# ZulutionAI/MoviiGen1.1

Measured on AMD Instinct MI355X. Metric: denoise-steps/sec, higher is better.
Workload: dtype bf16; 1 GPU; 14B T2V 1920x832x81f bf16 (the metric's configuration; BASELINE configs[2] shape); layers=40, parallelism=single, solver=unipc, weights=random N(0,0.02) bf16, seed 0

## Files before the change

### include/moviigen_hip.h

```cpp
#ifndef MOVIIGEN_HIP_H
#define MOVIIGEN_HIP_H

#include <stdint.h>

#ifdef __cplusplus
extern "C" {
#endif

#define MG_OK 0
#define MG_ERR_ARG (-1)
#define MG_ERR_SHAPE (-2)
#define MG_ERR_LAUNCH (-3)
#define MG_ERR_UNAVAILABLE (-4)
#define MG_ERR_COMM (-5)

const char* mg_version(void);
int mg_abi_version(void);


int mg_ln_modulate(const float* x, int64_t ldx, int64_t rows, int dim, const float* scale,
                   const float* shift, int add_one, float eps, int round_norm_bf16, void* out,
                   int out_f32, int64_t ldo, void* stream);

int64_t mg_step_resid_partials_bytes(void);
// ... 19 lines not shown

int mg_gemm_bf16(const uint16_t* A, int64_t lda, const uint16_t* W, int64_t ldw,
                 const float* bias, int64_t M, int N, int K, int epilogue, void* out,
                 int64_t ldo, const float* gate, void* stream);

int mg_quant_mxfp8_rows(const uint16_t* x, int64_t ldx, int64_t rows, int K, uint8_t* q, int64_t ldq,
                        uint8_t* scales, int64_t lds, void* stream);

int mg_gemm_mxfp8(const uint8_t* Aq, int64_t lda, const uint8_t* As, int64_t ldas, const uint8_t* Wq, int64_t ldw,
                  const uint8_t* Ws, int64_t ldws, const float* bias, int64_t M, int N, int K, int epilogue,
                  void* out, int64_t ldo, const float* gate, void* stream);

int mg_ln_modulate_mxfp8(const float* x, int64_t ldx, int64_t rows, int dim, const float* scale, const float* shift,
                         int add_one, float eps, int round_norm_bf16, uint16_t* out, int64_t ldo, uint8_t* q,
                         int64_t ldq, uint8_t* scales, int64_t lds, void* stream);

int mg_gemm_mxfp8_gelu_q(const uint8_t* Aq, int64_t lda, const uint8_t* As, int64_t ldas, const uint8_t* Wq, int64_t ldw,
                         const uint8_t* Ws, int64_t ldws, const float* bias, int64_t M, int N, int K, uint8_t* oq,
                         int64_t ldoq, uint8_t* oscales, int64_t ldos, void* stream);

int64_t mg_attn_workspace_bytes(void);
int mg_attn_fwd_bf16_hd128(const uint16_t* q, int64_t ldq, const uint16_t* kp, const uint16_t* vp,
                           uint16_t* o, int64_t ldo, int64_t Lq, int64_t Lk, int heads, float scale,
                           void* workspace, void* stream);

int mg_attn_fwd_bf16_hd128_lse(const uint16_t* q, int64_t ldq, const uint16_t* kp, const uint16_t* vp,
                               uint16_t* o, int64_t ldo, float* lse, int64_t Lq, int64_t Lk, int heads,
                               float scale, void* workspace, void* stream);

int mg_attn_fwd_bf16_hd128_prescaled(const uint16_t* q, int64_t ldq, const uint16_t* kp, const uint16_t* vp,
                                     uint16_t* o, int64_t ldo, float* lse, int64_t Lq, int64_t Lk, int heads,
                                     int reserve_cus, void* workspace, void* stream);

int mg_gate_residual_f32(float* x, int64_t ldx, const uint16_t* y, int64_t ldy, const float* gate, int64_t rows,
                         int dim, void* stream);


int mg_sp_pack_qkv_bf16(const uint16_t* q, int64_t ldq, const uint16_t* k, int64_t ldk, const uint16_t* v,
                        int64_t ldv, int64_t Lloc, int P, int cols_per_dest, int col0, int w, uint16_t* send,
                        void* stream);

int mg_sp_unpack_o_bf16(const uint16_t* recv, int64_t Lloc, int P, int cols_per_src, int col0, int w, uint16_t* o,
                        int64_t ldo, void* stream);

int mg_sp_copy_blocks_bf16(const uint16_t* src, int64_t s_blk, int64_t s_row, uint16_t* dst, int64_t d_blk,
                           int64_t d_row, int blocks, int64_t rows, int width, void* stream);


int mg_comm_unique_id(void* id128);
int mg_comm_create(const void* id128, int nranks, int rank, void** comm);
int mg_comm_destroy(void* comm);

int mg_sp_all_to_all(void* comm, const void* send, void* recv, int64_t bytes_per_peer, void* stream);

int mg_sp_all_to_all_4d_bf16(void* comm, const uint16_t* x, int64_t ldx, int64_t rows, int heads, int head_dim,
                             int seq_to_head, uint16_t* out, int64_t ldo, uint16_t* workspace, void* stream);

int mg_sp_all_gather(void* comm, const void* send, void* recv, int64_t bytes, void* stream);
int mg_shard_all_gather(void* comm, const void* shard, void* full, int64_t shard_bytes, void* stream);

int mg_attn_merge_f32(float* acc, int64_t lda, float* lse_acc, const uint16_t* part, int64_t ldp,
                      const float* lse_part, uint16_t* out, int64_t ldo, int64_t Lq, int heads, int first,
                      void* stream);

int mg_attn_fwd_bf16_generic(const uint16_t* q, int64_t ldq, const uint16_t* k, int64_t ldk,
                             const uint16_t* v, int64_t ldv, uint16_t* o, int64_t ldo, int64_t Lq,
// ... 112 lines not shown
```

### moviigen1.1_amd/csrc/attn_hd128.hip

```cpp
#include "common.h"
#include "../../include/moviigen_hip.h"

#define ATT_QB 256

__global__ __launch_bounds__(256) void pack_kv_kernel(const uint16_t* __restrict__ k, int64_t ldk,
                                                      const uint16_t* __restrict__ v, int64_t ldv, int64_t L,
                                                      uint16_t* __restrict__ kp, uint16_t* __restrict__ vp, int nt,
                                                      int korder) {
    __shared__ uint16_t tile[64][128 + 8];
    const int head = blockIdx.y, t = blockIdx.x;
    const int64_t k0 = (int64_t)t * 64;
    const int64_t tbase = ((int64_t)head * nt + t) * 8192;
    if (k) {
#pragma unroll
        for (int i = 0; i < 4; ++i) {
            const int id = threadIdx.x + i * 256;
            const int r = id >> 4, c = id & 15;
            u16x8_t u = {0, 0, 0, 0, 0, 0, 0, 0};
            if (k0 + r < L) u = *(const u16x8_t*)(k + (k0 + r) * ldk + head * 128 + c * 8);
            const int row = korder ? ((r & 32) | ((r & 4) << 2) | ((r & 24) >> 1) | (r & 3)) : r;
            *(u16x8_t*)(kp + tbase + c * 512 + row * 8) = u;
        }
    }
    if (v) {
#pragma unroll
        for (int i = 0; i < 4; ++i) {
            const int id = threadIdx.x + i * 256;
            const int r = id >> 4, c = id & 15;
            u16x8_t u = {0, 0, 0, 0, 0, 0, 0, 0};
            if (k0 + r < L) u = *(const u16x8_t*)(v + (k0 + r) * ldv + head * 128 + c * 8);
            *(u16x8_t*)&tile[r][c * 8] = u;
        }
        __syncthreads();
#pragma unroll
        for (int i = 0; i < 4; ++i) {
            const int id = threadIdx.x + i * 256;
            const int kc = id >> 7, d = id & 127;
            u16x8_t u;
#pragma unroll
            for (int j = 0; j < 8; ++j) u[j] = tile[kc * 8 + j][d];
            *(u16x8_t*)(vp + tbase + kc * 1024 + d * 8) = u;
        }
    }
}

#ifdef MG_AB_BUILD
int mg_attn_w64_launch(const uint16_t* q, int64_t ldq, const uint16_t* kp, const uint16_t* vp, uint16_t* o, int64_t ldo,
                       int64_t Lq, int64_t Lk, int heads, float c_log2, int nqb, float* lse, hipStream_t st);
#endif
int mg_attn_m16_launch(const uint16_t* q, int64_t ldq, const uint16_t* kp, const uint16_t* vp, uint16_t* o, int64_t ldo,
                       int64_t Lq, int64_t Lk, int heads, float c_log2, int prescaled, int nqb, float* lse, int reserve_cus,
                       unsigned* workspace, hipStream_t st);

#ifdef MG_AB_BUILD
static int g_attn_variant = 0;
extern "C" int mg_attn_set_variant(int v) {
    if (v != 0 && v != 3) return MG_ERR_ARG;
    g_attn_variant = v;
    return MG_OK;
}
#else
static constexpr int g_attn_variant = 0;
#endif

extern "C" int mg_pack_kv_bf16(const uint16_t* k, int64_t ldk, const uint16_t* v, int64_t ldv, int64_t L, int heads,
                               int head_dim, uint16_t* kp, uint16_t* vp, void* stream) {
    if ((!k && !v) || (k && !kp) || (v && !vp)) return MG_ERR_ARG;
    if (head_dim != 128 || heads <= 0 || L <= 0 || (k && (ldk & 7)) || (v && (ldv & 7))) return MG_ERR_SHAPE;
    const int nt = (int)((L + 63) / 64);
    hipLaunchKernelGGL(pack_kv_kernel, dim3(nt, heads), dim3(256), 0, (hipStream_t)stream, k, ldk, v, ldv, L, kp, vp,
                       nt, g_attn_variant == 3 ? 0 : 1);
    return mg_check_launch();
}

static int attn_fwd_impl(const uint16_t* q, int64_t ldq, const uint16_t* kp, const uint16_t* vp, uint16_t* o, int64_t ldo,
                         float* lse, int64_t Lq, int64_t Lk, int heads, float scale, int prescaled, int reserve_cus, void* workspace,
                         void* stream) {
    if (!q || !kp || !vp || !o) return MG_ERR_ARG;
    if ((uintptr_t)workspace & 7) return MG_ERR_SHAPE;
    if (Lq < 0 || Lk <= 0 || heads <= 0 || reserve_cus < 0) return MG_ERR_SHAPE;
    if ((ldq & 7) || (ldo & 3)) return MG_ERR_SHAPE;
    if (((uintptr_t)q & 15) || ((uintptr_t)kp & 15) || ((uintptr_t)vp & 15) || ((uintptr_t)o & 7)) return MG_ERR_SHAPE;
    if (Lq == 0) return MG_OK;
    const int64_t nqb64 = (Lq + ATT_QB - 1) / ATT_QB;
    if (nqb64 * heads > 0x7fffffffLL) return MG_ERR_SHAPE;
    const int nqb = (int)nqb64;
    const float c_log2 = scale * 1.4426950408889634f;
    hipStream_t st = (hipStream_t)stream;
#ifdef MG_AB_BUILD
    if (g_attn_variant == 3)
        return mg_attn_w64_launch(q, ldq, kp, vp, o, ldo, Lq, Lk, heads, prescaled ? 1.0f : c_log2, nqb, lse, st);
#endif
    return mg_attn_m16_launch(q, ldq, kp, vp, o, ldo, Lq, Lk, heads, c_log2, prescaled, nqb, lse, reserve_cus, (unsigned*)workspace, st);
}

extern "C" int64_t mg_attn_workspace_bytes(void) { return 256; }

extern "C" int mg_attn_fwd_bf16_hd128_lse(const uint16_t* q, int64_t ldq, const uint16_t* kp, const uint16_t* vp,
                                          uint16_t* o, int64_t ldo, float* lse, int64_t Lq, int64_t Lk, int heads,
                                          float scale, void* workspace, void* stream) {
    return attn_fwd_impl(q, ldq, kp, vp, o, ldo, lse, Lq, Lk, heads, scale, 0, 0, workspace, stream);
}
extern "C" int mg_attn_fwd_bf16_hd128(const uint16_t* q, int64_t ldq, const uint16_t* kp, const uint16_t* vp,
                                      uint16_t* o, int64_t ldo, int64_t Lq, int64_t Lk, int heads, float scale,
                                      void* workspace, void* stream) {
    return attn_fwd_impl(q, ldq, kp, vp, o, ldo, nullptr, Lq, Lk, heads, scale, 0, 0, workspace, stream);
}
extern "C" int mg_attn_fwd_bf16_hd128_prescaled(const uint16_t* q, int64_t ldq, const uint16_t* kp, const uint16_t* vp,
                                                uint16_t* o, int64_t ldo, float* lse, int64_t Lq, int64_t Lk, int heads,
                                                int reserve_cus, void* workspace, void* stream) {
    return attn_fwd_impl(q, ldq, kp, vp, o, ldo, lse, Lq, Lk, heads, 1.0f, 1, reserve_cus, workspace, stream);
}
```

### moviigen1.1_amd/csrc/attn_hd128_m16.hip

```cpp
#include <type_traits>
#include "common.h"
#include "../../include/moviigen_hip.h"

#define M16_THREADS 256
#define M16_QB 256
#define M16_TILE 16384
#define M16_K(slot) ((slot) * M16_TILE)
#define M16_V(slot) (3 * M16_TILE + (slot) * M16_TILE)

MG_DEV bf16x8_t m16_bf(u32x4_t v) { return __builtin_bit_cast(bf16x8_t, v); }
struct M16State {
    f32x4_t ot[8][4];
    f32x4_t st[2][2][4];
    bf16x8_t pf[2][4];
    f32x4_t mq[4];
    float m_run[4], l_run[4];
    float psa[4], psb[4];
    int bad;
};

template <int OFF>
MG_DEV void m16_rd(bf16x8_t& dst, unsigned addr) {
    asm volatile("ds_read_b128 %0, %1 offset:%2" : "=v"(dst) : "v"(addr), "i"(OFF));
}
// ... 702 lines not shown
#define M16_ORD 9
#define M16_LAUNCH(PROF, SCALED, ORD)                                                                                             \
    hipLaunchKernelGGL((attn_hd128_m16_kernel<PROF, SCALED, ORD>), dim3(grid), dim3(M16_THREADS), 0, st, q, ldq, kp, vp, o, ldo, Lq, \
                       Lk, heads, prescaled ? 1.0f : c_log2, nqb, g_m16_dbg, PROF ? g_m16_prof : nullptr, lse, g_m16_flagcnt, tickets)
#ifdef MG_AB_BUILD
    const int ord = (g_m16_dbg >> 1) & 7;
    const int mo = (g_m16_dbg >> 5) & 3;
    if (mo && prescaled && !g_m16_prof) {
        if (mo == 1) M16_LAUNCH(false, false, 8);
        else if (mo == 2) M16_LAUNCH(false, false, 9);
        else M16_LAUNCH(false, false, 1);
        return mg_check_launch();
    }
    if (ord && prescaled && !g_m16_prof) {
        if (ord == 1) M16_LAUNCH(false, false, 1);
        else if (ord == 2) M16_LAUNCH(false, false, 2);
        else if (ord == 3) M16_LAUNCH(false, false, 3);
        else if (ord == 4) M16_LAUNCH(false, false, 4);
        else if (ord == 5) M16_LAUNCH(false, false, 5);
        else M16_LAUNCH(false, false, 0);
        return mg_check_launch();
    }
#endif
    if (g_m16_prof) {
        if (prescaled) M16_LAUNCH(true, false, M16_ORD);
        else M16_LAUNCH(true, true, M16_ORD);
    } else {
        if (prescaled) M16_LAUNCH(false, false, M16_ORD);
        else M16_LAUNCH(false, true, M16_ORD);
    }
#undef M16_LAUNCH
    return mg_check_launch();
}
```

### moviigen1.1_amd/wan/backend/lib.py

```python
import ctypes
import os

_HERE = os.path.dirname(os.path.abspath(__file__))
LIB_PATH = os.path.normpath(os.path.join(_HERE, '..', '..', 'lib', 'libmoviigen_hip.so'))
LIB_AB_PATH = os.path.normpath(os.path.join(_HERE, '..', '..', 'lib', 'libmoviigen_hip_ab.so'))

c_i64, c_int, c_f32, c_vp = ctypes.c_int64, ctypes.c_int, ctypes.c_float, ctypes.c_void_p

SIGNATURES = {
    'mg_version': [],
    'mg_abi_version': [],
    'mg_ln_modulate': [c_vp, c_i64, c_i64, c_int, c_vp, c_vp, c_int, c_f32, c_int, c_vp, c_int, c_i64, c_vp],
    'mg_step_resid_partials_bytes': [],
    'mg_step_resid_capture_f32': [c_vp, c_vp, c_vp, c_i64, c_vp, c_vp, c_vp],
    'mg_resid_ln_modulate_f32': [c_vp, c_i64, c_vp, c_i64, c_i64, c_int, c_vp, c_vp, c_f32, c_vp, c_i64, c_vp],
    'mg_rmsnorm_rope_bf16': [c_vp, c_i64, c_vp, c_i64, c_i64, c_int, c_vp, c_f32, c_int, c_vp, c_int, c_int,
                             c_int, c_i64, c_f32, c_vp],
    'mg_pack_kv_bf16': [c_vp, c_i64, c_vp, c_i64, c_i64, c_int, c_int, c_vp, c_vp, c_vp],
    'mg_gemm_bf16': [c_vp, c_i64, c_vp, c_i64, c_vp, c_i64, c_int, c_int, c_int, c_vp, c_i64, c_vp, c_vp],
    'mg_quant_mxfp8_rows': [c_vp, c_i64, c_i64, c_int, c_vp, c_i64, c_vp, c_i64, c_vp],
    'mg_gemm_mxfp8': [c_vp, c_i64, c_vp, c_i64, c_vp, c_i64, c_vp, c_i64, c_vp, c_i64, c_int, c_int, c_int, c_vp, c_i64,
                      c_vp, c_vp],
    'mg_ln_modulate_mxfp8': [c_vp, c_i64, c_i64, c_int, c_vp, c_vp, c_int, c_f32, c_int, c_vp, c_i64, c_vp, c_i64, c_vp, c_i64, c_vp],
    'mg_gemm_mxfp8_gelu_q': [c_vp, c_i64, c_vp, c_i64, c_vp, c_i64, c_vp, c_i64, c_vp, c_i64, c_int, c_int, c_vp, c_i64, c_vp, c_i64,
                             c_vp],
    'mg_attn_workspace_bytes': [],
    'mg_attn_fwd_bf16_hd128': [c_vp, c_i64, c_vp, c_vp, c_vp, c_i64, c_i64, c_i64, c_int, c_f32, c_vp, c_vp],
    'mg_attn_fwd_bf16_hd128_lse': [c_vp, c_i64, c_vp, c_vp, c_vp, c_i64, c_vp, c_i64, c_i64, c_int, c_f32, c_vp, c_vp],
    'mg_attn_fwd_bf16_hd128_prescaled': [c_vp, c_i64, c_vp, c_vp, c_vp, c_i64, c_vp, c_i64, c_i64, c_int, c_int, c_vp, c_vp],
    'mg_attn_merge_f32': [c_vp, c_i64, c_vp, c_vp, c_i64, c_vp, c_vp, c_i64, c_i64, c_int, c_int, c_vp],
    'mg_attn_fwd_bf16_generic': [c_vp, c_i64, c_vp, c_i64, c_vp, c_i64, c_vp, c_i64, c_i64, c_i64, c_int, c_int,
                                 c_f32, c_vp],
    'mg_sinusoid_embed': [c_vp, c_int, c_int, c_int, c_vp, c_vp],
    'mg_gemv_f32': [c_vp, c_vp, c_vp, c_vp, c_int, c_int, c_int, c_vp],
    'mg_add_rows_f32': [c_vp, c_vp, c_vp, c_int, c_int, c_int, c_vp],
    'mg_head_gemm_f32': [c_vp, c_i64, c_vp, c_vp, c_vp, c_i64, c_int, c_int, c_vp],
    'mg_patchify_bf16': [c_vp, c_int, c_int, c_int, c_int, c_int, c_int, c_vp, c_i64, c_vp],
    'mg_unpatchify_f32': [c_vp, c_i64, c_int, c_int, c_int, c_int, c_int, c_int, c_vp, c_vp],
    'mg_lincomb4_f32': [c_vp, c_i64, c_vp, c_f32, c_vp, c_f32, c_vp, c_f32, c_vp, c_f32, c_vp],
    'mg_cfg_combine_f32': [c_vp, c_vp, c_vp, c_f32, c_i64, c_vp],
    'mg_embed_rows_bf16': [c_vp, c_i64, c_int, c_vp, c_int, c_vp, c_vp],
    'mg_ew_bf16': [c_vp, c_vp, c_vp, c_i64, c_int, c_vp],
    'mg_t5_attn_bf16': [c_vp, c_vp, c_vp, c_i64, c_vp, c_vp, c_vp, c_i64, c_i64, c_i64, c_int, c_int, c_vp],
    'mg_vae_conv_f32': [c_vp, c_vp, c_int, c_int, c_int, c_int, c_int, c_vp, c_vp, c_int, c_int, c_int, c_int,
                        c_int, c_vp, c_vp, c_int, c_vp],
    'mg_vae_upconv_fold_weights_f32': [c_vp, c_int, c_int, c_vp, c_vp],
    'mg_vae_upconv_phases_f32': [c_vp, c_int, c_int, c_int, c_int, c_vp, c_vp, c_int, c_vp, c_int, c_vp],
    'mg_vae_conv_cols_f32': [c_vp, c_vp, c_int, c_int, c_int, c_int, c_int, c_vp, c_vp, c_int, c_int, c_int, c_int,
                             c_vp, c_vp, c_int, c_int, c_int, c_vp],
    'mg_vae_upconv_phases_cols_f32': [c_vp, c_int, c_int, c_int, c_int, c_vp, c_vp, c_int, c_vp, c_int, c_int, c_int, c_vp],
    'mg_vae_rmsnorm_silu_f32': [c_vp, c_vp, c_vp, c_i64, c_int, c_int, c_vp],
    'mg_vae_attn_workspace_floats': [c_i64, c_int],
    'mg_vae_attn_f32': [c_vp, c_vp, c_int, c_i64, c_int, c_vp, c_vp],
    'mg_vae_attn_rows_f32': [c_vp, c_i64, c_vp, c_vp, c_i64, c_vp, c_int, c_i64, c_i64, c_int, c_vp, c_vp],
    'mg_vae_latent_in_f32': [c_vp, c_vp, c_vp, c_int, c_int, c_int, c_int, c_vp, c_vp],
    'mg_vae_video_out_f32': [c_vp, c_int, c_int, c_int, c_int, c_vp, c_int, c_int, c_vp],
    'mg_vae_time_interleave_f32': [c_vp, c_int, c_i64, c_int, c_vp, c_vp],
    'mg_vae_conv_strided_f32': [c_vp, c_vp, c_int, c_int, c_int, c_int, c_int, c_vp, c_vp, c_int, c_int, c_int, c_int,
                                c_int, c_int, c_int, c_int, c_int, c_int, c_int, c_int, c_vp, c_int, c_vp],
    'mg_vae_conv_in3_f32': [c_vp, c_vp, c_int, c_int, c_int, c_int, c_vp, c_vp, c_int, c_vp, c_int, c_vp],
    'mg_vae_video_in_f32': [c_vp, c_int, c_int, c_int, c_int, c_int, c_vp, c_vp],
    'mg_vae_latent_out_f32': [c_vp, c_int, c_vp, c_vp, c_int, c_int, c_int, c_int, c_vp, c_vp],
# ... 101 lines not shown
```

### moviigen1.1_amd/wan/backend/ops.py

```python
import ctypes

import torch

from . import lib

BIAS_BF16, BIAS_GELU_BF16, GATE_RESID_F32, BIAS_F32 = 0, 1, 2, 3


def _p(t):
    return None if t is None else ctypes.c_void_p(t.data_ptr())


def _st():
    return ctypes.c_void_p(torch.cuda.current_stream().cuda_stream)


def _epilogue_dtype(epilogue):
    return torch.bfloat16 if epilogue in (BIAS_BF16, BIAS_GELU_BF16) else torch.float32


def _chk(t, dtype, name):
    if t is None:
        return
    if not t.is_cuda:
# ... 113 lines not shown
                                   f'wq{tuple(wq.shape)} w_scales{tuple(w_scales.shape)} out{tuple(out.shape)}')
    lib.call('mg_gemm_mxfp8', _p(aq), aq.stride(0), _p(a_scales), a_scales.stride(0), _p(wq), wq.stride(0), _p(w_scales),
             w_scales.stride(0), _p(bias), M, N, K, int(epilogue), _p(out), out.stride(0), _p(gate), _st())
    return out


def ln_modulate_mxfp8(x, scale, shift, add_one, eps, q, scales, out=None, round_norm_bf16=False):
    _chk(x, torch.float32, 'x'); _chk(scale, torch.float32, 'scale'); _chk(shift, torch.float32, 'shift')
    _chk(q, torch.uint8, 'q'); _chk(scales, torch.uint8, 'scales'); _chk(out, torch.bfloat16, 'out')
    rows, dim = x.shape
    if tuple(q.shape) != (rows, dim) or tuple(scales.shape) != (rows, dim // 32) or (out is not None and tuple(out.shape) != (rows, dim)):
        raise lib.MoviigenHipError(f'ln_modulate_mxfp8 shape mismatch x{tuple(x.shape)} q{tuple(q.shape)} scales{tuple(scales.shape)}')
    lib.call('mg_ln_modulate_mxfp8', _p(x), x.stride(0), rows, dim, _p(scale), _p(shift), int(add_one), float(eps),
             int(round_norm_bf16), _p(out), 0 if out is None else out.stride(0), _p(q), q.stride(0), _p(scales), scales.stride(0), _st())
    return q, scales


def gemm_mxfp8_gelu_q(aq, a_scales, wq, w_scales, bias, oq, o_scales):
    _chk(aq, torch.uint8, 'aq'); _chk(a_scales, torch.uint8, 'a_scales'); _chk(wq, torch.uint8, 'wq')
    _chk(w_scales, torch.uint8, 'w_scales'); _chk(bias, torch.float32, 'bias'); _chk(oq, torch.uint8, 'oq')
    _chk(o_scales, torch.uint8, 'o_scales')
    M, K = aq.shape
    N = wq.shape[0]
    if (wq.shape[1] != K or tuple(oq.shape) != (M, N) or tuple(o_scales.shape) != (M, N // 32)
            or tuple(a_scales.shape) != (M, K // 32) or tuple(w_scales.shape) != (N, K // 32)):
        raise lib.MoviigenHipError(f'gemm_mxfp8_gelu_q shape mismatch aq{tuple(aq.shape)} a_scales{tuple(a_scales.shape)} '
                                   f'wq{tuple(wq.shape)} w_scales{tuple(w_scales.shape)} oq{tuple(oq.shape)} o_scales{tuple(o_scales.shape)}')
    lib.call('mg_gemm_mxfp8_gelu_q', _p(aq), aq.stride(0), _p(a_scales), a_scales.stride(0), _p(wq), wq.stride(0), _p(w_scales),
             w_scales.stride(0), _p(bias), M, N, K, _p(oq), oq.stride(0), _p(o_scales), o_scales.stride(0), _st())
    return oq, o_scales


_ATTN_WS = {}


def attention_workspace(device=None, stream=None):
    dev = torch.cuda.current_device() if device is None else torch.device(device).index
    st = torch.cuda.current_stream(dev) if stream is None else stream
    key = (dev, st.cuda_stream)
    ws = _ATTN_WS.get(key)
    if ws is None:
        with torch.cuda.stream(st):
            ws = torch.zeros(int(lib.load().mg_attn_workspace_bytes()), dtype=torch.uint8, device=f'cuda:{dev}')
        _ATTN_WS[key] = ws
    return ws


def attention_hd128(q, kp, vp, out, lk, heads, scale, prescaled=False, reserve_cus=0, workspace='stream', lse=None):
    _chk(q, torch.bfloat16, 'q'); _chk(kp, torch.bfloat16, 'kp'); _chk(vp, torch.bfloat16, 'vp')
    _chk(out, torch.bfloat16, 'out'); _chk(lse, torch.float32, 'lse')
    if min(kp.numel(), vp.numel()) < packed_kv_numel(int(lk), int(heads)):
        raise lib.MoviigenHipError('packed K/V buffers too small for lk keys')
    if lse is not None and (lse.numel() < int(heads) * q.shape[0] or not lse.is_contiguous()):
        raise lib.MoviigenHipError('lse must be a contiguous [heads, Lq] fp32 tensor')
    ws = attention_workspace(q.device) if isinstance(workspace, str) else workspace
    head = (_p(q), q.stride(0), _p(kp), _p(vp), _p(out), out.stride(0))
    if prescaled:
        lib.call('mg_attn_fwd_bf16_hd128_prescaled', *head, _p(lse), q.shape[0], int(lk), int(heads), int(reserve_cus), _p(ws), _st())
    elif lse is not None:
        lib.call('mg_attn_fwd_bf16_hd128_lse', *head, _p(lse), q.shape[0], int(lk), int(heads), float(scale), _p(ws), _st())
    else:
        lib.call('mg_attn_fwd_bf16_hd128', *head, q.shape[0], int(lk), int(heads), float(scale), _p(ws), _st())
    return out


_attention_hd128 = attention_hd128


def attention_hd128_lse(q, kp, vp, out, lse, lk, heads, scale, prescaled=False):
    return _attention_hd128(q, kp, vp, out, lk, heads, scale, prescaled=prescaled, lse=lse), lse


def attention_generic(q, k, v, out, lk, heads, head_dim, scale):
    _chk(q, torch.bfloat16, 'q'); _chk(k, torch.bfloat16, 'k'); _chk(v, torch.bfloat16, 'v')
    _chk(out, torch.bfloat16, 'out')
    lib.call('mg_attn_fwd_bf16_generic', _p(q), q.stride(0), _p(k), k.stride(0), _p(v), v.stride(0), _p(out),
             out.stride(0), q.shape[0], int(lk), int(heads), int(head_dim), float(scale), _st())
    return out


def sinusoid_embed(t, dim, out):
    code = {torch.int64: 0, torch.float32: 1, torch.float64: 2}.get(t.dtype)
    if code is None or not t.is_cuda:
        raise lib.MoviigenHipError('timestep must be a CUDA int64/float32/float64 tensor')
    lib.call('mg_sinusoid_embed', _p(t), code, t.numel(), int(dim), _p(out), _st())
    return out


def gemv(w, bias, x, y, silu_in=False):
    _chk(w, torch.float32, 'w'); _chk(x, torch.float32, 'x'); _chk(y, torch.float32, 'y')
    lib.call('mg_gemv_f32', _p(w), _p(bias), _p(x), _p(y), w.shape[0], w.shape[1], int(silu_in), _st())
# ... 326 lines not shown
```

### moviigen1.1_amd/wan/modules/attention.py

```python
import math

import torch

from ..backend import ops

__all__ = ['flash_attention', 'attention']


def q_prescale(head_dim):
    return ops.ATTN_LOG2E / math.sqrt(head_dim) if head_dim == 128 else 1.0


def pack_tiles(k, v, klen, heads, tiles=None):
    if tiles is None:
        n_pk = ops.packed_kv_numel(klen, heads)
        tiles = tuple(torch.empty(n_pk, dtype=torch.bfloat16, device=k.device) for _ in range(2))
    ops.pack_kv(k[:klen], v[:klen], heads, tiles[0], tiles[1])
    return tiles


def attend(q, k, v, out, klen, heads, head_dim, scale=None, prescaled=True, packed=False, tiles=None, reserve_cus=0):
    scale = 1.0 / math.sqrt(head_dim) if scale is None else scale
    if head_dim != 128:
        return ops.attention_generic(q, k, v, out, klen, heads, head_dim, scale)
    if not packed:
        k, v = pack_tiles(k, v, klen, heads, tiles)
    return ops.attention_hd128(q, k, v, out, klen, heads, scale, prescaled=prescaled, reserve_cus=reserve_cus)


def flash_attention(q, k, v, q_lens=None, k_lens=None, dropout_p=0., softmax_scale=None, q_scale=None,
                    causal=False, window_size=(-1, -1), deterministic=False, dtype=torch.bfloat16, version=None):
    assert dtype == torch.bfloat16, 'the MI355X kernels are bf16'
    assert q.is_cuda and q.size(-1) <= 256
    if causal or dropout_p != 0. or tuple(window_size) != (-1, -1):
        raise NotImplementedError('causal / dropout / window attention are never used by the reference DiT')
    b, lq, n, c = q.shape
    lk = k.size(1)
    assert k.size(2) == n and v.size(2) == n, 'grouped-query attention is not used by the reference DiT'
    out_dtype = q.dtype
    if q_scale is not None:
        q = q * q_scale
    scale = softmax_scale if softmax_scale is not None else 1.0 / math.sqrt(c)
    out = torch.zeros(b, lq, n, c, dtype=torch.bfloat16, device=q.device)
    for i in range(b):
        ql = lq if q_lens is None else int(q_lens[i])
        kl = lk if k_lens is None else int(k_lens[i])
        qi = q[i, :ql].to(torch.bfloat16).reshape(ql, n * c).contiguous()
        ki = k[i, :kl].to(torch.bfloat16).reshape(kl, n * c).contiguous()
        vi = v[i, :kl].to(torch.bfloat16).reshape(kl, n * c).contiguous()
        oi = torch.empty(ql, n * c, dtype=torch.bfloat16, device=q.device)
        attend(qi, ki, vi, oi, kl, n, c, scale=scale, prescaled=False)
        out[i, :ql] = oi.view(ql, n, c)
    return out.type(out_dtype)


def attention(q, k, v, q_lens=None, k_lens=None, dropout_p=0., softmax_scale=None, q_scale=None, causal=False,
              window_size=(-1, -1), deterministic=False, dtype=torch.bfloat16, fa_version=None):
    return flash_attention(q=q, k=k, v=v, q_lens=q_lens, k_lens=k_lens, dropout_p=dropout_p,
                           softmax_scale=softmax_scale, q_scale=q_scale, causal=causal, window_size=window_size,
                           deterministic=deterministic, dtype=dtype, version=fa_version)
# ... 1 lines not shown
```

Before: 0.04491 steps/s.

## Add short-key attention kernel keeping all K tiles resident in LDS

Adds a persistent attention kernel for key lengths up to 512 (cross-attention to text tokens) that loads every K tile of a head into shared memory once and reuses it across the query blocks of that head, streaming only V through a double buffer. Work items are split across XCDs, and the next item's Q is prefetched during the tail of the current one. The prescaled entry now dispatches to this kernel automatically when Lk is at most 512. The cost is a large new hand-scheduled kernel with inline buffer-to-LDS asm and an exact fallback path for overflowed softmax sums.

Result: no change. 0.04498 steps/s (median of 6 runs) (+0.2%).

```diff
diff --git a/include/moviigen_hip.h b/include/moviigen_hip.h
--- a/include/moviigen_hip.h
+++ b/include/moviigen_hip.h
@@ -75,6 +75,13 @@
                                      uint16_t* o, int64_t ldo, float* lse, int64_t Lq, int64_t Lk, int heads,
                                      int reserve_cus, void* workspace, void* stream);
 
+int mg_attn_fwd_bf16_hd128_shortk(const uint16_t* q, int64_t ldq, const uint16_t* kp, const uint16_t* vp,
+                                  uint16_t* o, int64_t ldo, float* lse, int64_t Lq, int64_t Lk, int heads,
+                                  int reserve_cus, void* stream);
+int mg_attn_fwd_bf16_hd128_prescaled_generic(const uint16_t* q, int64_t ldq, const uint16_t* kp, const uint16_t* vp,
+                                             uint16_t* o, int64_t ldo, float* lse, int64_t Lq, int64_t Lk, int heads,
+                                             int reserve_cus, void* workspace, void* stream);
+
 int mg_gate_residual_f32(float* x, int64_t ldx, const uint16_t* y, int64_t ldy, const float* gate, int64_t rows,
                          int dim, void* stream);
 
diff --git a/moviigen1.1_amd/csrc/attn_hd128.hip b/moviigen1.1_amd/csrc/attn_hd128.hip
--- a/moviigen1.1_amd/csrc/attn_hd128.hip
+++ b/moviigen1.1_amd/csrc/attn_hd128.hip
@@ -51,6 +51,9 @@
 int mg_attn_m16_launch(const uint16_t* q, int64_t ldq, const uint16_t* kp, const uint16_t* vp, uint16_t* o, int64_t ldo,
                        int64_t Lq, int64_t Lk, int heads, float c_log2, int prescaled, int nqb, float* lse, int reserve_cus,
                        unsigned* workspace, hipStream_t st);
+int mg_attn_shortk_launch(const uint16_t* q, int64_t ldq, const uint16_t* kp, const uint16_t* vp, uint16_t* o, int64_t ldo, int64_t Lq, int64_t Lk,
+                          int heads, int nqb, float* lse, int reserve_cus, hipStream_t st);
+#define ATT_SHORT_KEYS 512
 
 #ifdef MG_AB_BUILD
 static int g_attn_variant = 0;
@@ -75,7 +78,7 @@
 
 static int attn_fwd_impl(const uint16_t* q, int64_t ldq, const uint16_t* kp, const uint16_t* vp, uint16_t* o, int64_t ldo,
                          float* lse, int64_t Lq, int64_t Lk, int heads, float scale, int prescaled, int reserve_cus, void* workspace,
-                         void* stream) {
+                         void* stream, int short_keys = 0) {
     if (!q || !kp || !vp || !o) return MG_ERR_ARG;
     if ((uintptr_t)workspace & 7) return MG_ERR_SHAPE;
     if (Lq < 0 || Lk <= 0 || heads <= 0 || reserve_cus < 0) return MG_ERR_SHAPE;
@@ -87,6 +90,11 @@
     const int nqb = (int)nqb64;
     const float c_log2 = scale * 1.4426950408889634f;
     hipStream_t st = (hipStream_t)stream;
+    if (short_keys < 0) short_keys = prescaled && Lk <= ATT_SHORT_KEYS && g_attn_variant == 0;
+    if (short_keys) {
+        if (!prescaled || Lk > ATT_SHORT_KEYS || g_attn_variant != 0) return MG_ERR_SHAPE;
+        return mg_attn_shortk_launch(q, ldq, kp, vp, o, ldo, Lq, Lk, heads, nqb, lse, reserve_cus, st);
+    }
 #ifdef MG_AB_BUILD
     if (g_attn_variant == 3)
         return mg_attn_w64_launch(q, ldq, kp, vp, o, ldo, Lq, Lk, heads, prescaled ? 1.0f : c_log2, nqb, lse, st);
@@ -109,5 +117,15 @@
 extern "C" int mg_attn_fwd_bf16_hd128_prescaled(const uint16_t* q, int64_t ldq, const uint16_t* kp, const uint16_t* vp,
                                                 uint16_t* o, int64_t ldo, float* lse, int64_t Lq, int64_t Lk, int heads,
                                                 int reserve_cus, void* workspace, void* stream) {
-    return attn_fwd_impl(q, ldq, kp, vp, o, ldo, lse, Lq, Lk, heads, 1.0f, 1, reserve_cus, workspace, stream);
+    return attn_fwd_impl(q, ldq, kp, vp, o, ldo, lse, Lq, Lk, heads, 1.0f, 1, reserve_cus, workspace, stream, -1);
 }
+extern "C" int mg_attn_fwd_bf16_hd128_prescaled_generic(const uint16_t* q, int64_t ldq, const uint16_t* kp, const uint16_t* vp,
+                                                        uint16_t* o, int64_t ldo, float* lse, int64_t Lq, int64_t Lk, int heads,
+                                                        int reserve_cus, void* workspace, void* stream) {
+    return attn_fwd_impl(q, ldq, kp, vp, o, ldo, lse, Lq, Lk, heads, 1.0f, 1, reserve_cus, workspace, stream, 0);
+}
+extern "C" int mg_attn_fwd_bf16_hd128_shortk(const uint16_t* q, int64_t ldq, const uint16_t* kp, const uint16_t* vp,
+                                             uint16_t* o, int64_t ldo, float* lse, int64_t Lq, int64_t Lk, int heads,
+                                             int reserve_cus, void* stream) {
+    return attn_fwd_impl(q, ldq, kp, vp, o, ldo, lse, Lq, Lk, heads, 1.0f, 1, reserve_cus, nullptr, stream, 1);
+}
diff --git a/moviigen1.1_amd/csrc/attn_hd128_m16.hip b/moviigen1.1_amd/csrc/attn_hd128_m16.hip
--- a/moviigen1.1_amd/csrc/attn_hd128_m16.hip
+++ b/moviigen1.1_amd/csrc/attn_hd128_m16.hip
@@ -758,3 +758,387 @@
 #undef M16_LAUNCH
     return mg_check_launch();
 }
+
+#define SK_MAXT 8
+#define SK_K(t) ((t) * M16_TILE)
+#define SK_V(slot) (SK_MAXT * M16_TILE + (slot) * M16_TILE)
+typedef __attribute__((address_space(3))) char* sk_lds_t;
+
+template <int KB>
+MG_DEV void sk_bare_S(M16State& s, const bf16x8_t (&qf)[4][4], sk_lds_t ktile, int lim, int G, int qi) {
+    const f32x4_t zero4[4] = {{0.f, 0.f, 0.f, 0.f}, {0.f, 0.f, 0.f, 0.f}, {0.f, 0.f, 0.f, 0.f}, {0.f, 0.f, 0.f, 0.f}};
+    if (lim < 64) m16_mask_init<KB>(s, lim, G, zero4);
+    else {
+#pragma unroll
+        for (int blk = 0; blk < 2; ++blk)
+#pragma unroll
+            for (int n = 0; n < 4; ++n) s.st[KB][blk][n] = (f32x4_t){0.f, 0.f, 0.f, 0.f};
+    }
+    const sk_lds_t base = ktile + G * 1024 + qi * 16 + KB * 512;
+#pragma unroll
+    for (int i = 0; i < 8; ++i) {
+        const bf16x8_t f = *(const __attribute__((address_space(3))) bf16x8_t*)(base + m16_koff(i));
+#pragma unroll
+        for (int n = 0; n < 4; ++n)
+            s.st[KB][i >> 2][n] = __builtin_amdgcn_mfma_f32_16x16x32_bf16(f, qf[n][i & 3], s.st[KB][i >> 2][n], 0, 0, 0);
+    }
+}
+template <int KB>
+MG_DEV void sk_bare_PV(M16State& s, const char* vtile, int G, int qi) {
+    const char* base = vtile + G * 2048 + qi * 16 + KB * 8192;
+#pragma unroll
+    for (int i = 0; i < 8; ++i) {
+        const bf16x8_t f = *(const bf16x8_t*)(base + m16_voff(i));
+#pragma unroll
+        for (int n = 0; n < 4; ++n)
+            s.ot[i][n] = __builtin_amdgcn_mfma_f32_16x16x32_bf16(f, s.pf[KB][n], s.ot[i][n], 0, 0, 0);
+    }
+}
+MG_DEV void sk_reset(M16State& s) {
+#pragma unroll
+    for (int d = 0; d < 8; ++d)
+#pragma unroll
+        for (int n = 0; n < 4; ++n) s.ot[d][n] = (f32x4_t){0.f, 0.f, 0.f, 0.f};
+#pragma unroll
+    for (int n = 0; n < 4; ++n) s.m_run[n] = -1e30f, s.l_run[n] = 0.f, s.psa[n] = 0.f, s.psb[n] = 0.f;
+    s.bad = 0;
+}
+MG_DEV void sk_load_q(bf16x8_t (&qf)[4][4], const uint16_t* __restrict__ q, int64_t ldq, int64_t Lq, int head, int qb0, int wave, int G, int qi) {
+    const int64_t qrow_base = (int64_t)qb0 * M16_QB + wave * 64 + qi;
+#pragma unroll
+    for (int n = 0; n < 4; ++n) {
+        const int64_t qr = qrow_base + n * 16;
+        const int64_t qrow = qr < Lq ? qr : Lq - 1;
+        const uint16_t* qp = q + qrow * ldq + head * 128 + G * 8;
+#pragma unroll
+        for (int c = 0; c < 4; ++c) qf[n][c] = m16_bf(*(const u32x4_t*)(qp + c * 32));
+    }
+}
+MG_DEV void sk_store_o(const M16State& s, uint16_t* __restrict__ o, int64_t ldo, float* __restrict__ lse, int64_t Lq, int head, int qb0, int wave, int G, int qi,
+                       bool wide) {
+#pragma unroll
+    for (int n = 0; n < 4; ++n) {
+        float l_tot = s.l_run[n] + __shfl_xor(s.l_run[n], 16, 64);
+        l_tot += __shfl_xor(l_tot, 32, 64);
+        const float inv = 1.f / l_tot;
+        const int64_t qr = (int64_t)qb0 * M16_QB + wave * 64 + n * 16 + qi;
+        if (lse && G == 0 && qr < Lq) lse[(int64_t)head * Lq + qr] = (s.m_run[n] * 1.0f + __log2f(l_tot)) * 0.6931471805599453f;
+        uint2 pk[8];
+#pragma unroll
+        for (int d = 0; d < 8; ++d) {
+            pk[d].x = pack_bf2(s.ot[d][n][0] * inv, s.ot[d][n][1] * inv);
+            pk[d].y = pack_bf2(s.ot[d][n][2] * inv, s.ot[d][n][3] * inv);
+        }
+        if (wide) {
+            uint4 v[4];
+#pragma unroll
+            for (int j = 0; j < 4; ++j) {
+                const auto x = __builtin_amdgcn_permlane16_swap(pk[2 * j].x, pk[2 * j + 1].x, false, false);
+                const auto y = __builtin_amdgcn_permlane16_swap(pk[2 * j].y, pk[2 * j + 1].y, false, false);
+                v[j] = make_uint4(x[0], y[0], x[1], y[1]);
+            }
+            if (qr < Lq) {
+                uint16_t* op = o + qr * ldo + head * 128 + (G & 1) * 16 + (G >> 1) * 8;
+#pragma unroll
+                for (int j = 0; j < 4; ++j) *(uint4*)(op + j * 32) = v[j];
+            }
+        } else if (qr < Lq) {
+            uint16_t* op = o + qr * ldo + head * 128 + G * 4;
+#pragma unroll
+            for (int d = 0; d < 8; ++d) *(uint2*)(op + d * 16) = pk[d];
+        }
+    }
+}
+template <int N>
+MG_DEV void sk_dma(const u32x4_t& rs, int voff, int soff, unsigned dst) {
+    if (N == 4)
+        asm volatile("s_mov_b32 m0, %2\n\ts_nop 4\n\t"
+                     "buffer_load_dwordx4 %0, %1, %3 offen lds\n\t"
+                     "buffer_load_dwordx4 %0, %1, %3 offen offset:1024 lds\n\t"
+                     "buffer_load_dwordx4 %0, %1, %3 offen offset:2048 lds\n\t"
+                     "buffer_load_dwordx4 %0, %1, %3 offen offset:3072 lds"
+                     :: "v"(voff), "s"(rs), "s"(dst), "s"(soff) : "memory");
+    else
+        asm volatile("s_mov_b32 m0, %2\n\ts_nop 4\n\t"
+                     "buffer_load_dwordx4 %0, %1, %3 offen lds\n\t"
+                     "buffer_load_dwordx4 %0, %1, %3 offen offset:1024 lds"
+                     :: "v"(voff), "s"(rs), "s"(dst), "s"(soff) : "memory");
+}
+MG_DEV u32x4_t sk_resource(const void* base, unsigned bytes) {
+    const uint64_t b = (uint64_t)(uintptr_t)base;
+    return (u32x4_t){(unsigned)__builtin_amdgcn_readfirstlane((int)(unsigned)b), (unsigned)__builtin_amdgcn_readfirstlane((int)((unsigned)(b >> 32) & 0xffffu)),
+                     bytes, 0x00020000u};
+}
+
+static __device__ __noinline__ void sk_exact_block(const uint16_t* __restrict__ q, int64_t ldq, const uint16_t* __restrict__ vp,
+                                                   uint16_t* __restrict__ o, int64_t ldo, float* __restrict__ lse, int64_t Lq, int head, int qb0,
+                                                   int T, int last_lim, sk_lds_t smem3) {
+    const int wave = __builtin_amdgcn_readfirstlane((int)threadIdx.x >> 6);
+    const int lane = m16_lane();
+    const int qi = lane & 15, G = lane >> 4;
+    bf16x8_t qf[4][4];
+    sk_load_q(qf, q, ldq, Lq, head, qb0, wave, G, qi);
+    M16State s;
+    sk_reset(s);
+    for (int t = 0; t < T; ++t) {
+        const int lim = t == T - 1 ? last_lim : 64;
+        const char* vtile = (const char*)(vp + ((int64_t)head * T + t) * 8192);
+        sk_bare_S<0>(s, qf, smem3 + SK_K(t), lim, G, qi);
+        sk_bare_S<1>(s, qf, smem3 + SK_K(t), lim, G, qi);
+        m16_softmax_exact<0>(s, 1.0f);
+        sk_bare_PV<0>(s, vtile, G, qi);
+        m16_softmax_exact<1>(s, 1.0f);
+        sk_bare_PV<1>(s, vtile, G, qi);
+    }
+    sk_store_o(s, o, ldo, lse, Lq, head, qb0, wave, G, qi, ((ldo & 7) == 0) && (((uintptr_t)o & 15) == 0));
+}
+
+template <bool PROF, bool RAGGED>
+__global__ __launch_bounds__(M16_THREADS, 1) void attn_hd128_shortk_kernel(
+    const uint16_t* __restrict__ q, int64_t ldq, const uint16_t* __restrict__ kp, const uint16_t* __restrict__ vp,
+    uint16_t* __restrict__ o, int64_t ldo, int64_t Lq, int64_t Lk, int heads, int nqb, int dbg,
+    unsigned long long* __restrict__ prof, float* __restrict__ lse, unsigned* __restrict__ flagcnt) {
+    __shared__ __attribute__((aligned(16))) char smem[(SK_MAXT + 2) * M16_TILE];
+    constexpr int ORD = 9;
+    const int bid = blockIdx.x, nwg = gridDim.x, tid = threadIdx.x;
+    const int wave = __builtin_amdgcn_readfirstlane(tid >> 6);
+    const int total_items = nqb * heads;
+    int item, item_end;
+    if (nwg & 7) {
+        item = (int)((int64_t)bid * total_items / nwg), item_end = (int)((int64_t)(bid + 1) * total_items / nwg);
+    } else {
+        const int xcd = bid & 7, slot = bid >> 3, per = nwg >> 3;
+        const int x0 = (int)((int64_t)xcd * total_items / 8), xn = (int)((int64_t)(xcd + 1) * total_items / 8) - x0;
+        item = x0 + (int)((int64_t)slot * xn / per), item_end = x0 + (int)((int64_t)(slot + 1) * xn / per);
+    }
+    if (item >= item_end) return;
+    const int T = (int)((Lk + 63) / 64);
+    const int last_lim = (int)(Lk - (int64_t)(T - 1) * 64);
+    const int nfull = RAGGED ? T - 1 : T;
+    const bool pipelined = nfull >= 3;
+    const bool wide_o = ((ldo & 7) == 0) && (((uintptr_t)o & 15) == 0);
+    const sk_lds_t smem3 = (sk_lds_t)smem;
+    const unsigned lds0 = (unsigned)(uintptr_t)(mg_lptr_t)smem;
+    const unsigned kvbytes = (unsigned)heads * (unsigned)T * M16_TILE;
+    const u32x4_t rs_k = sk_resource(kp, kvbytes), rs_v = sk_resource(vp, kvbytes);
+    unsigned long long ph[8] = {0, 0, 0, 0, 0, 0, 0, 0}, ph_t = 0, pf_fence = 0, pf_step = 0, pf_n = 0;
+    int p = 0;
+    int cur_head = -1;
+    bf16x8_t qf[4][4];
+    if (pipelined) {
+        const int l0 = m16_lane();
+        sk_load_q(qf, q, ldq, Lq, item / nqb, item % nqb, wave, l0 >> 4, l0 & 15);
+    }
+    auto fence = [&]() __attribute__((always_inline)) {
+        asm volatile("s_waitcnt vmcnt(0)" ::: "memory");
+        __syncthreads();
+    };
+    auto fence_hot = [&]() __attribute__((always_inline)) { asm volatile("s_waitcnt vmcnt(0)\n\ts_barrier" ::: "memory"); };
+    while (item < item_end) {
+        const int head = item / nqb;
+        const int qb0 = item - head * nqb;
+        const int lane = m16_lane();
+        int qi = lane & 15, G = lane >> 4;
+        const int hb = head * T * M16_TILE;
+        const bool has_next = item + 1 < item_end;
+        const int nitem = has_next ? item + 1 : item;
+        const int nhb = has_next ? ((item + 1) / nqb) * T * M16_TILE : 0;
+        const int dvo2 = wave * 2048 + lane * 16;
+        const unsigned lds_vw = (unsigned)__builtin_amdgcn_readfirstlane((int)(lds0 + SK_V(0) + wave * 2048));
+        auto req = [&](int h) __attribute__((always_inline)) {
+            if (h >= 2 * T && !has_next) return;
+            const int off = h < 2 * T ? hb + h * 8192 : nhb + (h - 2 * T) * 8192;
+            sk_dma<2>(rs_v, dvo2, __builtin_amdgcn_readfirstlane(off), lds_vw + (unsigned)(((p + (h >> 1)) & 1) * M16_TILE + (h & 1) * 8192));
+        };
+        if (PROF) ph_t = __builtin_amdgcn_s_memtime();
+        if (head != cur_head) {
+            __syncthreads();
+            const int dvo4 = wave * 4096 + lane * 16;
+            for (int t = 0; t < T; ++t)
+                sk_dma<4>(rs_k, dvo4, __builtin_amdgcn_readfirstlane(hb + t * M16_TILE), (unsigned)__builtin_amdgcn_readfirstlane((int)(lds0 + SK_K(t) + wave * 4096)));
+            if (cur_head < 0 && pipelined) req(0), req(1), req(2), req(3);
+            fence();
+            cur_head = head;
+        }
+        if (!pipelined) {
+            sk_exact_block(q, ldq, vp, o, ldo, lse, Lq, head, qb0, T, last_lim, smem3);
+            ++item;
+            continue;
+        }
+        unsigned kbase = lds0 + G * 1024 + qi * 16;
+        unsigned vbase = lds0 + SK_V(0) + G * 2048 + qi * 16;
+        auto k_addr = [&](int t, int kb) __attribute__((always_inline)) { return kbase + t * M16_TILE + kb * 512; };
+        auto v_addr = [&](int t, int kb) __attribute__((always_inline)) { return vbase + ((p + t) & 1) * M16_TILE + kb * 8192; };
+#pragma unroll
+        for (int n = 0; n < 4; ++n)
+#pragma unroll
+            for (int c = 0; c < 4; ++c) asm volatile("" : "+a"(qf[n][c]));
+        M16State s;
+        bf16x8_t kf[4], vf[4];
+        sk_reset(s);
+        sk_bare_S<0>(s, qf, smem3 + SK_K(0), 64, G, qi);
+        sk_bare_S<1>(s, qf, smem3 + SK_K(0), 64, G, qi);
+#pragma unroll
+        for (int n = 0; n < 4; ++n) {
+            const float a = fmaxf(fmaxf(s.st[0][0][n][0], s.st[0][0][n][1]), fmaxf(s.st[0][0][n][2], s.st[0][0][n][3]));
+            const float b = fmaxf(fmaxf(s.st[0][1][n][0], s.st[0][1][n][1]), fmaxf(s.st[0][1][n][2], s.st[0][1][n][3]));
+            const float c2 = fmaxf(fmaxf(s.st[1][0][n][0], s.st[1][0][n][1]), fmaxf(s.st[1][0][n][2], s.st[1][0][n][3]));
+            const float d2 = fmaxf(fmaxf(s.st[1][1][n][0], s.st[1][1][n][1]), fmaxf(s.st[1][1][n][2], s.st[1][1][n][3]));
+            float m = fmaxf(-1e30f, fmaxf(fmaxf(a, b), fmaxf(c2, d2)));
+            m = fmaxf(m, __shfl_xor(m, 16, 64));
+            m = fmaxf(m, __shfl_xor(m, 32, 64)) + 64.f;
+            s.mq[n] = (f32x4_t){-m, -m, -m, -m};
+        }
+#pragma unroll
+        for (int kb = 0; kb < 2; ++kb)
+#pragma unroll
+            for (int blk = 0; blk < 2; ++blk)
+#pragma unroll
+                for (int n = 0; n < 4; ++n) s.st[kb][blk][n] += s.mq[n];
+        m16_softmax_zero<0>(s, 1.0f);
+#pragma unroll
+        for (int n = 0; n < 4; ++n) asm volatile("" : "+v"(s.l_run[n]));
+        m16_rd<m16_koff(0)>(kf[0], k_addr(1, 0));
+        m16_rd<m16_voff(0)>(vf[0], v_addr(0, 0));
+        m16_rd<m16_koff(1)>(kf[1], k_addr(1, 0));
+        m16_rd<m16_voff(1)>(vf[1], v_addr(0, 0));
+        m16_step<0, 1, true, true, false, ORD>(s, qf, kf, vf, k_addr(1, 0), v_addr(0, 0), k_addr(1, 1), v_addr(0, 1), 1.0f, M16NoDma());
+        int t = 1;
+        unsigned ka = k_addr(1, 0);
+        unsigned va0 = v_addr(0, 0), va1 = v_addr(1, 0);
+        unsigned lvA = lds_vw + (unsigned)(((p + t + 1) & 1) * M16_TILE), lvB = lds_vw + (unsigned)(((p + t) & 1) * M16_TILE);
+        int offa = __builtin_amdgcn_readfirstlane(hb + (t + 1) * M16_TILE), offb = __builtin_amdgcn_readfirstlane(hb + (t + 1) * M16_TILE + 8192);
+        unsigned keep_m0, rot_tmp;
+#define SK_BDMA0(VOFF, RS, SOFF, LBASE, IMM)                                                                                               \
+    asm volatile("s_add_u32 m0, %2, %3\n\ts_nop 0\n\tbuffer_load_dwordx4 %0, %1, %4 offen lds"                                             \
+                 :: "v"(VOFF), "s"(RS), "s"(LBASE), "n"(IMM), "s"(SOFF) : "memory", "scc")
+#define SK_BDMAN(VOFF, RS, SOFF, IMM)                                                                                                      \
+    asm volatile("buffer_load_dwordx4 %0, %1, %3 offen offset:%2 lds" :: "v"(VOFF), "s"(RS), "n"(IMM), "s"(SOFF) : "memory")
+        asm volatile("s_mov_b32 %0, m0\n\ts_nop 4" : "=s"(keep_m0) :: "memory");
+        if (PROF) { const unsigned long long tt = __builtin_amdgcn_s_memtime(); ph[0] += tt - ph_t; ph_t = tt; }
+        __builtin_amdgcn_s_waitcnt(0x0F70);
+        asm volatile("" : "+v"(ka), "+v"(va0), "+v"(va1));
+        for (; t + 1 < nfull; ++t) {
+            const unsigned long long c0 = PROF ? __builtin_amdgcn_s_memtime() : 0;
+            fence_hot();
+            const unsigned long long c1 = PROF ? __builtin_amdgcn_s_memtime() : 0;
+            m16_step<1, 1, true, true, false, ORD, 512, 8192, M16_TILE, 0>(s, qf, kf, vf, ka, va0, ka, va1, 1.0f,
+                                       [&](int n) __attribute__((always_inline)) {
+                                           if (n == 0) SK_BDMA0(dvo2, rs_v, offa, lvA, 0);
+                                           else if (n == 1) SK_BDMAN(dvo2, rs_v, offa, 1024);
+                                       });
+            const unsigned long long c2 = PROF ? __builtin_amdgcn_s_memtime() : 0;
+            fence_hot();
+            const unsigned long long c3 = PROF ? __builtin_amdgcn_s_memtime() : 0;
+            m16_step<0, 1, true, true, false, ORD, M16_TILE, 0, M16_TILE + 512, 8192>(s, qf, kf, vf, ka, va1, ka, va1, 1.0f,
+                                       [&](int n) __attribute__((always_inline)) {
+                                           if (n == 0) SK_BDMA0(dvo2, rs_v, offb, lvA, 8192);
+                                           else if (n == 1) SK_BDMAN(dvo2, rs_v, offb, 1024);
+                                           else if (n == 2)
+                                               asm volatile("s_add_u32 %0, %0, 0x4000\n\ts_add_u32 %1, %1, 0x4000" : "+s"(offa), "+s"(offb) : : "scc");
+                                           else if (n == 3)
+                                               asm volatile("s_mov_b32 %2, %0\n\ts_mov_b32 %0, %1\n\ts_mov_b32 %1, %2" : "+s"(lvA), "+s"(lvB), "=&s"(rot_tmp));
+                                           else if (n == 7)
+                                               asm volatile("v_add_u32 %0, 0x4000, %0\n\tv_swap_b32 %1, %2" : "+v"(ka), "+v"(va0), "+v"(va1));
+                                       });
+            if (PROF) {
+                const unsigned long long c4 = __builtin_amdgcn_s_memtime();
+                pf_fence += (c1 - c0) + (c3 - c2), pf_step += (c2 - c1) + (c4 - c3), pf_n += 1;
+            }
+        }
+#undef SK_BDMA0
+#undef SK_BDMAN
+        asm volatile("s_mov_b32 m0, %0" :: "s"(keep_m0) : "memory");
+        if (PROF) { const unsigned long long tt = __builtin_amdgcn_s_memtime(); ph[1] += tt - ph_t; ph_t = tt; }
+        static_assert(M16_TILE == 0x4000, "the literals above");
+        {
+            const int l2 = m16_lane();
+            qi = l2 & 15, G = l2 >> 4;
+            kbase = lds0 + G * 1024 + qi * 16;
+            vbase = lds0 + SK_V(0) + G * 2048 + qi * 16;
+        }
+        int u = 2 * t;
+        fence(), req(u + 2), ++u;
+        m16_step<1, 1, true, true, false, ORD>(s, qf, kf, vf, k_addr(t, 1), v_addr(t - 1, 1), k_addr(t + 1, 0), v_addr(t, 0), 1.0f, M16NoDma());
+        if constexpr (RAGGED) {
+            fence(), req(u + 2), ++u;
+            m16_mask_init<0>(s, last_lim, G, s.mq);
+            m16_step<0, 2, true, true, false, ORD>(s, qf, kf, vf, k_addr(t + 1, 0), v_addr(t, 0), k_addr(t + 1, 1), v_addr(t, 1), 1.0f, M16NoDma());
+            fence(), req(u + 2), ++u;
+            m16_mask_init<1>(s, last_lim, G, s.mq);
+            m16_step<1, 2, true, true, false, ORD>(s, qf, kf, vf, k_addr(t + 1, 1), v_addr(t, 1), k_addr(t + 1, 1), v_addr(t + 1, 0), 1.0f, M16NoDma());
+            fence(), req(u + 2), ++u;
+            m16_step<0, 0, true, true, false, ORD>(s, qf, kf, vf, k_addr(t + 1, 1), v_addr(t + 1, 0), k_addr(t + 1, 1), v_addr(t + 1, 1), 1.0f, M16NoDma());
+            ++u;
+            asm volatile("s_waitcnt vmcnt(0)" ::: "memory");
+            sk_load_q(qf, q, ldq, Lq, nitem / nqb, nitem % nqb, wave, G, qi);
+            m16_step<1, 0, true, false, false, ORD>(s, qf, kf, vf, k_addr(t + 1, 1), v_addr(t + 1, 1), k_addr(t + 1, 1), v_addr(t + 1, 1), 1.0f, M16NoDma());
+        } else {
+            fence(), req(u + 2), ++u;
+            m16_step<0, 0, true, true, false, ORD>(s, qf, kf, vf, k_addr(t, 1), v_addr(t, 0), k_addr(t, 1), v_addr(t, 1), 1.0f, M16NoDma());
+            ++u;
+            asm volatile("s_waitcnt vmcnt(0)" ::: "memory");
+            sk_load_q(qf, q, ldq, Lq, nitem / nqb, nitem % nqb, wave, G, qi);
+            m16_step<1, 0, true, false, false, ORD>(s, qf, kf, vf, k_addr(t, 1), v_addr(t, 1), k_addr(t, 1), v_addr(t, 1), 1.0f, M16NoDma());
+        }
+        m16_wait<0>();
+        asm volatile("" ::"v"(kf[0]), "v"(kf[1]), "v"(kf[2]), "v"(kf[3]), "v"(vf[0]), "v"(vf[1]), "v"(vf[2]), "v"(vf[3]));
+#pragma unroll
+        for (int n = 0; n < 4; ++n) {
+            s.l_run[n] += s.psa[n] + s.psb[n];
+            s.psa[n] = s.psb[n] = 0.f;
+            float lt = s.l_run[n] + __shfl_xor(s.l_run[n], 16, 64);
+            lt += __shfl_xor(lt, 32, 64);
+            s.bad |= !(lt >= 8.4703295e-22f && lt <= 1.2379400e27f);
+            s.m_run[n] = -s.mq[n][0];
+        }
+        if (PROF) { const unsigned long long tt = __builtin_amdgcn_s_memtime(); ph[2] += tt - ph_t; ph_t = tt; }
+        __syncthreads();
+        req(u + 1), req(u + 2);
+        if (PROF) { const unsigned long long tt = __builtin_amdgcn_s_memtime(); ph[3] += tt - ph_t; ph_t = tt; }
+        {
+            const int l3 = m16_lane();
+            qi = l3 & 15, G = l3 >> 4;
+        }
+        p = (p + T) & 1;
+        if (__any(s.bad) && !(dbg & 1)) {
+            if (flagcnt && (tid & 63) == 0) atomicAdd(flagcnt + 1, 1u);
+            sk_exact_block(q, ldq, vp, o, ldo, lse, Lq, head, qb0, T, last_lim, smem3);
+        } else
+            sk_store_o(s, o, ldo, lse, Lq, head, qb0, wave, G, qi, wide_o);
+        if (PROF) { const unsigned long long tt = __builtin_amdgcn_s_memtime(); ph[4] += tt - ph_t; ph[6] += 1; }
+        ++item;
+    }
+    if (PROF && prof && (tid & 63) == 0) {
+        atomicAdd(prof + wave * 4 + 0, pf_fence);
+        atomicAdd(prof + wave * 4 + 1, pf_step);
+        atomicAdd(prof + wave * 4 + 3, pf_n);
+    }
+    if (PROF && prof && tid == 0) {
+#pragma unroll
+        for (int i = 0; i < 8; ++i) atomicAdd(prof + 1040 + i, ph[i]);
+    }
+}
+
+int mg_attn_shortk_launch(const uint16_t* q, int64_t ldq, const uint16_t* kp, const uint16_t* vp, uint16_t* o, int64_t ldo, int64_t Lq, int64_t Lk,
+                          int heads, int nqb, float* lse, int reserve_cus, hipStream_t st) {
+    if (Lk > 64 * SK_MAXT) return MG_ERR_SHAPE;
+    if ((int64_t)heads * ((Lk + 63) / 64) * M16_TILE > 0x7fffffffLL) return MG_ERR_SHAPE;
+    const int n_cu = mg_persistent_cus(reserve_cus);
+    if (n_cu < 0) return MG_ERR_LAUNCH;
+    const int total = nqb * heads;
+    const unsigned grid = total <= n_cu ? (unsigned)total : (unsigned)n_cu;
+#define SK_LAUNCH(PROF, RAGGED)                                                                                                          \
+    hipLaunchKernelGGL((attn_hd128_shortk_kernel<PROF, RAGGED>), dim3(grid), dim3(M16_THREADS), 0, st, q, ldq, kp, vp, o, ldo, Lq, Lk, heads, nqb, \
+                       g_m16_dbg, PROF ? g_m16_prof : nullptr, lse, g_m16_flagcnt)
+    const bool ragged = (Lk & 63) != 0;
+    if (g_m16_prof) {
+        if (ragged) SK_LAUNCH(true, true);
+        else SK_LAUNCH(true, false);
+    } else {
+        if (ragged) SK_LAUNCH(false, true);
+        else SK_LAUNCH(false, false);
+    }
+#undef SK_LAUNCH
+    return mg_check_launch();
+}
diff --git a/moviigen1.1_amd/wan/backend/lib.py b/moviigen1.1_amd/wan/backend/lib.py
--- a/moviigen1.1_amd/wan/backend/lib.py
+++ b/moviigen1.1_amd/wan/backend/lib.py
@@ -28,6 +28,8 @@
     'mg_attn_fwd_bf16_hd128': [c_vp, c_i64, c_vp, c_vp, c_vp, c_i64, c_i64, c_i64, c_int, c_f32, c_vp, c_vp],
     'mg_attn_fwd_bf16_hd128_lse': [c_vp, c_i64, c_vp, c_vp, c_vp, c_i64, c_vp, c_i64, c_i64, c_int, c_f32, c_vp, c_vp],
     'mg_attn_fwd_bf16_hd128_prescaled': [c_vp, c_i64, c_vp, c_vp, c_vp, c_i64, c_vp, c_i64, c_i64, c_int, c_int, c_vp, c_vp],
+    'mg_attn_fwd_bf16_hd128_prescaled_generic': [c_vp, c_i64, c_vp, c_vp, c_vp, c_i64, c_vp, c_i64, c_i64, c_int, c_int, c_vp, c_vp],
+    'mg_attn_fwd_bf16_hd128_shortk': [c_vp, c_i64, c_vp, c_vp, c_vp, c_i64, c_vp, c_i64, c_i64, c_int, c_int, c_vp],
     'mg_attn_merge_f32': [c_vp, c_i64, c_vp, c_vp, c_i64, c_vp, c_vp, c_i64, c_i64, c_int, c_int, c_vp],
     'mg_attn_fwd_bf16_generic': [c_vp, c_i64, c_vp, c_i64, c_vp, c_i64, c_vp, c_i64, c_i64, c_i64, c_int, c_int,
                                  c_f32, c_vp],
diff --git a/moviigen1.1_amd/wan/backend/ops.py b/moviigen1.1_amd/wan/backend/ops.py
--- a/moviigen1.1_amd/wan/backend/ops.py
+++ b/moviigen1.1_amd/wan/backend/ops.py
@@ -169,6 +169,7 @@
 
 
 _ATTN_WS = {}
+SHORT_KEYS = 512
 
 
 def attention_workspace(device=None, stream=None):
@@ -183,7 +184,7 @@
     return ws
 
 
-def attention_hd128(q, kp, vp, out, lk, heads, scale, prescaled=False, reserve_cus=0, workspace='stream', lse=None):
+def attention_hd128(q, kp, vp, out, lk, heads, scale, prescaled=False, reserve_cus=0, workspace='stream', lse=None, short_keys=None):
     _chk(q, torch.bfloat16, 'q'); _chk(kp, torch.bfloat16, 'kp'); _chk(vp, torch.bfloat16, 'vp')
     _chk(out, torch.bfloat16, 'out'); _chk(lse, torch.float32, 'lse')
     if min(kp.numel(), vp.numel()) < packed_kv_numel(int(lk), int(heads)):
@@ -192,8 +193,13 @@
         raise lib.MoviigenHipError('lse must be a contiguous [heads, Lq] fp32 tensor')
     ws = attention_workspace(q.device) if isinstance(workspace, str) else workspace
     head = (_p(q), q.stride(0), _p(kp), _p(vp), _p(out), out.stride(0))
-    if prescaled:
-        lib.call('mg_attn_fwd_bf16_hd128_prescaled', *head, _p(lse), q.shape[0], int(lk), int(heads), int(reserve_cus), _p(ws), _st())
+    if short_keys is not None and not prescaled:
+        raise lib.MoviigenHipError('short_keys selects a kernel of the pre-scaled entry only')
+    if prescaled and short_keys:
+        lib.call('mg_attn_fwd_bf16_hd128_shortk', *head, _p(lse), q.shape[0], int(lk), int(heads), int(reserve_cus), _st())
+    elif prescaled:
+        entry = 'mg_attn_fwd_bf16_hd128_prescaled' if short_keys is None else 'mg_attn_fwd_bf16_hd128_prescaled_generic'
+        lib.call(entry, *head, _p(lse), q.shape[0], int(lk), int(heads), int(reserve_cus), _p(ws), _st())
     elif lse is not None:
         lib.call('mg_attn_fwd_bf16_hd128_lse', *head, _p(lse), q.shape[0], int(lk), int(heads), float(scale), _p(ws), _st())
     else:
diff --git a/moviigen1.1_amd/wan/modules/attention.py b/moviigen1.1_amd/wan/modules/attention.py
--- a/moviigen1.1_amd/wan/modules/attention.py
+++ b/moviigen1.1_amd/wan/modules/attention.py
@@ -19,13 +19,14 @@
     return tiles
 
 
-def attend(q, k, v, out, klen, heads, head_dim, scale=None, prescaled=True, packed=False, tiles=None, reserve_cus=0):
+def attend(q, k, v, out, klen, heads, head_dim, scale=None, prescaled=True, packed=False, tiles=None, reserve_cus=0, short_keys=None):
     scale = 1.0 / math.sqrt(head_dim) if scale is None else scale
     if head_dim != 128:
         return ops.attention_generic(q, k, v, out, klen, heads, head_dim, scale)
     if not packed:
         k, v = pack_tiles(k, v, klen, heads, tiles)
-    return ops.attention_hd128(q, k, v, out, klen, heads, scale, prescaled=prescaled, reserve_cus=reserve_cus)
+    kw = {} if short_keys is None else {'short_keys': short_keys}
+    return ops.attention_hd128(q, k, v, out, klen, heads, scale, prescaled=prescaled, reserve_cus=reserve_cus, **kw)
 
 
 def flash_attention(q, k, v, q_lens=None, k_lens=None, dropout_p=0., softmax_scale=None, q_scale=None,
```
